# MecatronicaUSB/uwimageproc

Hardware: NVIDIA B200
Metric: chain_frames_per_s_4k (higher is better)
Workload: dtype u8 (histretch, aclahe) / int32+f64 (bgdehaze)

## Files before the change

### uwimageproc_b200/csrc/dehaze.cu

```cuda
#include <algorithm>

#include "common.cuh"

__global__ void fs_reset_kernel(FrameState* fs, int n) {
  int i = blockIdx.x * blockDim.x + threadIdx.x;
  if (i >= n) return;
  FrameState s;
  memset(&s, 0, sizeof(s));
  s.kmin = 255; s.kmax = 0;
  s.jmin_key[0] = s.jmin_key[1] = ~0ull;
  s.jmax_key[0] = s.jmax_key[1] = 0ull;
  s.rmin = 255; s.rmax = 0;
  s.yi_min = s.yj_min = 255; s.yi_max = s.yj_max = 0;
  s.omin_key = ~0ull; s.omax_key = 0ull;
  fs[i] = s;
}
int frame_state_reset(uwip_ctx* ctx, FrameState* fs, int n) {
  UWIP_LAUNCH(ctx, "fs_reset", fs_reset_kernel, cdiv(n, 128), 128, 0, fs, n);
  return UWIP_OK;
}
FrameState* frame_state_get(uwip_ctx* ctx, int n) { return (FrameState*)uwip_slot(ctx, SLOT_FSTATE, sizeof(FrameState) * (size_t)n); }

#include "gfmarch.cuh"

// ... 141 lines not shown
constexpr int WF_VR = WF_TY / 4, WF_CTAS = 3;
constexpr int WF_RB = 8;
constexpr int WF_PP = 84;
constexpr int WF_HP = 68;
constexpr int WF_HN = 16;

template <int N, bool MAX, int OFF, int M>
__device__ __forceinline__ void win15(const uint32_t (&p)[M], uint32_t (&o)[N]) {
  static_assert(OFF + N + 14 <= M, "window run");
  uint32_t a[N + 12], b[N + 6];
#pragma unroll
  for (int i = 0; i < N + 12; i++)
    a[i] = MAX ? __vimax3_u16x2(p[OFF + i], p[OFF + i + 1], p[OFF + i + 2]) : __vimin3_u16x2(p[OFF + i], p[OFF + i + 1], p[OFF + i + 2]);
#pragma unroll
  for (int i = 0; i < N + 6; i++) b[i] = MAX ? __vimax3_u16x2(a[i], a[i + 3], a[i + 6]) : __vimin3_u16x2(a[i], a[i + 3], a[i + 6]);
#pragma unroll
  for (int i = 0; i < N; i++) o[i] = MAX ? __vmaxu2(b[i], b[i + 6]) : __vminu2(b[i], b[i + 6]);
}

__device__ __forceinline__ void wf_cp_async8(void* smem, const void* gmem) {
  asm volatile("cp.async.ca.shared.global [%0], [%1], 8;" ::"r"((uint32_t)__cvta_generic_to_shared(smem)), "l"(gmem) : "memory");
}

template <bool FAST>
__device__ __forceinline__ uint32_t wf_emit_rows(const uint32_t (&mx0)[WF_VR], const uint32_t (&mx1)[WF_VR], const uint32_t (&mn0)[WF_VR],
                                                 const uint32_t* __restrict__ pc0, const uint32_t* __restrict__ pc1,
                                                 uint32_t* __restrict__ kqp, uint8_t* __restrict__ mgq, unsigned Wp, int nrows, int gy0, int H,
                                                 bool xt, bool inside, uint32_t km2) {
  uint32_t dmin2 = 0xffffffffu;
#pragma unroll
  for (int i = 0; i < WF_VR; i++) {
    if (!FAST && i >= nrows) break;
    const unsigned o = (unsigned)i * Wp;
    if (!FAST && !inside) { kqp[o] = 0u; mgq[o] = 0; continue; }
    const uint32_t t0 = pc0[i * WF_PP] - km2, t1 = pc1[i * WF_PP] - km2;
    uint32_t tn = mn0[i] - km2;
    if (!FAST) {
      const int gy = gy0 + i;
      if (xt || gy < WF_R || gy + WF_R >= H) tn = 0u;
    }
    kqp[o] = __byte_perm(__byte_perm(t0, t1, 0x4420), tn, 0x4210);
    mgq[o] = (uint8_t)(tn >> 16);
    dmin2 = __vminu2(dmin2, mx1[i] + 0x01000100u - mx0[i]);
  }
  return dmin2;
}

template <int CH>
__device__ __forceinline__ void wf_exact(const uint32_t (&mx0)[WF_VR], const uint32_t (&mx1)[WF_VR], int nrows, uint32_t target, int kmin,
                                         const double* s_nrm, unsigned idx0, unsigned W, double& bd, unsigned& bi) {
#pragma unroll
  for (int i = 0; i < WF_VR; i++) {
    if (i >= nrows) break;
    const uint32_t mr = mx1[i] & 0xffffu, mc = CH ? (mx0[i] >> 16) : (mx0[i] & 0xffffu);
    if (mr + 256u - mc == target) {
      const double d = s_nrm[mr - kmin] - s_nrm[mc - kmin];
      if (d < bd) { bd = d; bi = idx0 + (unsigned)i * W; }
    }
  }
}

__global__ void __launch_bounds__(256, WF_CTAS) window15_kernel(const uint8_t* __restrict__ src, int W, int H, int Wp,
                                                          const FrameState* __restrict__ fs, uint32_t* __restrict__ kq,
                                                          uint8_t* __restrict__ mgp, ArgPartial* __restrict__ partials) {
  extern __shared__ __align__(16) uint32_t s_w[];
  __shared__ double s_nrm[256];
  __shared__ uint32_t s_wmin[8];
  __shared__ int s_cnt[2];
  uint32_t* P0 = s_w;
  uint32_t* P1 = P0 + WF_RH * WF_PP;
  uint32_t* HX0 = P1 + WF_RH * WF_PP;
  uint32_t* HX1 = HX0 + WF_RH * WF_HP;
  uint32_t* HN0 = HX1 + WF_RH * WF_HP;
  const int f = blockIdx.z, tid = threadIdx.x, lane = tid & 31, warp = tid >> 5;
  const uint8_t* img = src + (size_t)f * W * H * 3;
  const int x0 = blockIdx.x * WF_TX, y0 = blockIdx.y * WF_TY;
  const int kmin = fs[f].kmin, range = (int)fs[f].kmax - kmin;
  s_nrm[tid] = (double)tid / (double)range;
  if (tid < 2) s_cnt[tid] = 0;
  uint32_t* RAW = HX0;
  const bool words = ((W & 3) == 0) && ((reinterpret_cast<uintptr_t>(img) & 3) == 0);
  const bool dwords = ((W & 7) == 0) && ((reinterpret_cast<uintptr_t>(img) & 7) == 0);
  if (dwords && x0 >= WF_RB && x0 - WF_RB + 80 <= W) {
    const uint2* col = reinterpret_cast<const uint2*>(img + (size_t)(x0 - WF_RB) * 3);
#pragma unroll
    for (int k = 0; k < (WF_RH + 7) / 8; k++) {
      const int ry = warp + 8 * k;
      if (ry < WF_RH && lane < 30) {
        const int y = min(max(y0 - WF_R + ry, 0), H - 1);
        wf_cp_async8(reinterpret_cast<uint2*>(RAW + ry * 64) + lane, col + (size_t)y * (W * 3 / 8) + lane);
      }
    }
    asm volatile("cp.async.wait_all;" ::: "memory");
    __syncthreads();
    for (int t = tid; t < WF_RH * 20; t += 256) {
      const int ry = t / 20, g = t - ry * 20;
      const uint32_t* w = RAW + ry * 64 + 3 * g;
      const uint32_t w0 = w[0], w1 = w[1], w2 = w[2];
      uint4 bg, rr;
      bg.x = __byte_perm(w0, 0u, 0x4140); bg.y = __byte_perm(w0, w1, 0x0403) & 0x00ff00ffu;
      bg.z = __byte_perm(w1, 0u, 0x4342); bg.w = __byte_perm(w2, 0u, 0x4241);
      rr.x = __byte_perm(w0, 0u, 0x4242); rr.y = __byte_perm(w1, 0u, 0x4141);
      rr.z = __byte_perm(w2, 0u, 0x4040); rr.w = __byte_perm(w2, 0u, 0x4343);
      *reinterpret_cast<uint4*>(P0 + ry * WF_PP + 4 * g) = bg;
      *reinterpret_cast<uint4*>(P1 + ry * WF_PP + 4 * g) = rr;
    }
  } else if (words) {
    const int xa = max(x0 - WF_RB, 0), xb = min(x0 - WF_RB + 79, W - 1);
    const int byte0 = (xa * 3) & ~3;
    const int nw = ((xb * 3 + 2) >> 2) - (byte0 >> 2) + 1;
#pragma unroll 4
    for (int idx = tid; idx < WF_RH * 64; idx += 256) {
      const int ry = idx >> 6, wi = idx & 63;
      if (wi < nw) {
        const int y = min(max(y0 - WF_R + ry, 0), H - 1);
        RAW[idx] = __ldg(reinterpret_cast<const uint32_t*>(img + (size_t)y * W * 3 + byte0) + wi);
      }
    }
    __syncthreads();
    if (tid < 240) {
      const int rx = tid % 80, rr = tid / 80;
      const int xc = min(max(x0 - WF_RB + rx, 0), W - 1);
      const uint8_t* rawb = reinterpret_cast<const uint8_t*>(RAW) + (xc * 3 - byte0);
#pragma unroll 7
      for (int ry = rr; ry < WF_RH; ry += 3) {
        const uint8_t* p = rawb + ry * 256;
        uint32_t b = p[0], g = p[1], r = p[2];
        P0[ry * WF_PP + rx] = b | (g << 16);
        P1[ry * WF_PP + rx] = r | (r << 16);
      }
    }
  } else if (tid < 240) {
    const int rx = tid % 80, rr = tid / 80;
    const int xc = min(max(x0 - WF_RB + rx, 0), W - 1);
    const uint8_t* col = img + (size_t)xc * 3;
#pragma unroll 7
    for (int ry = rr; ry < WF_RH; ry += 3) {
      const int y = min(max(y0 - WF_R + ry, 0), H - 1);
      const uint8_t* p = col + (size_t)y * W * 3;
      uint32_t b = __ldg(p), g = __ldg(p + 1), r = __ldg(p + 2);
      P0[ry * WF_PP + rx] = b | (g << 16);
      P1[ry * WF_PP + rx] = r | (r << 16);
    }
  }
  __syncthreads();
  if (tid < WF_RH * (WF_TX / WF_HN)) {
    const int ry = tid % WF_RH, j = tid / WF_RH;
    uint32_t p[WF_HN + 16], o[WF_HN];
    const uint4* r0 = reinterpret_cast<const uint4*>(P0 + ry * WF_PP + WF_HN * j);
#pragma unroll
    for (int q = 0; q < (WF_HN + 16) / 4; q++) { const uint4 v = r0[q]; p[4 * q] = v.x; p[4 * q + 1] = v.y; p[4 * q + 2] = v.z; p[4 * q + 3] = v.w; }
    win15<WF_HN, true, 1>(p, o);
    uint4* h0 = reinterpret_cast<uint4*>(HX0 + ry * WF_HP + WF_HN * j);
#pragma unroll
    for (int q = 0; q < WF_HN / 4; q++) h0[q] = make_uint4(o[4 * q], o[4 * q + 1], o[4 * q + 2], o[4 * q + 3]);
    win15<WF_HN, false, 1>(p, o);
    uint4* hn = reinterpret_cast<uint4*>(HN0 + ry * WF_HP + WF_HN * j);
#pragma unroll
    for (int q = 0; q < WF_HN / 4; q++) hn[q] = make_uint4(o[4 * q], o[4 * q + 1], o[4 * q + 2], o[4 * q + 3]);
    const uint4* r1 = reinterpret_cast<const uint4*>(P1 + ry * WF_PP + WF_HN * j);
#pragma unroll
    for (int q = 0; q < (WF_HN + 16) / 4; q++) { const uint4 v = r1[q]; p[4 * q] = v.x; p[4 * q + 1] = v.y; p[4 * q + 2] = v.z; p[4 * q + 3] = v.w; }
    win15<WF_HN, true, 1>(p, o);
    uint4* h1 = reinterpret_cast<uint4*>(HX1 + ry * WF_HP + WF_HN * j);
#pragma unroll
    for (int q = 0; q < WF_HN / 4; q++) h1[q] = make_uint4(o[4 * q], o[4 * q + 1], o[4 * q + 2], o[4 * q + 3]);
  }
  __syncthreads();
  const int x = tid & 63, run = tid >> 6;
  const int gx = x0 + x, ry0 = run * WF_VR, gy0 = y0 + ry0;
  const int nrows = gx < Wp ? min(WF_VR, H - gy0) : 0;
  const bool inside = gx < W;
  uint32_t mx0[WF_VR], mx1[WF_VR], dmin2 = 0xffffffffu;
  if (nrows > 0) {
    uint32_t p[WF_VR + 14], mn0[WF_VR];
#pragma unroll
    for (int i = 0; i < WF_VR + 14; i++) p[i] = HX0[(ry0 + i) * WF_HP + x];
    win15<WF_VR, true, 0>(p, mx0);
#pragma unroll
    for (int i = 0; i < WF_VR + 14; i++) p[i] = HX1[(ry0 + i) * WF_HP + x];
    win15<WF_VR, true, 0>(p, mx1);
#pragma unroll
    for (int i = 0; i < WF_VR + 14; i++) p[i] = HN0[(ry0 + i) * WF_HP + x];
    win15<WF_VR, false, 0>(p, mn0);
    const size_t pix0 = (size_t)f * Wp * H + (size_t)gy0 * Wp + gx;
    const uint32_t* pc0 = P0 + (ry0 + WF_R) * WF_PP + x + WF_RB;
    const uint32_t* pc1 = P1 + (ry0 + WF_R) * WF_PP + x + WF_RB;
    const uint32_t km2 = (uint32_t)kmin * 0x10001u;
    const bool xt = (gx < WF_R) || (gx + WF_R >= W);
    if (!xt && gy0 >= WF_R && gy0 + WF_VR - 1 + WF_R < H)
      dmin2 = wf_emit_rows<true>(mx0, mx1, mn0, pc0, pc1, kq + pix0, mgp + pix0, (unsigned)Wp, nrows, gy0, H, xt, inside, km2);
    else
      dmin2 = wf_emit_rows<false>(mx0, mx1, mn0, pc0, pc1, kq + pix0, mgp + pix0, (unsigned)Wp, nrows, gy0, H, xt, inside, km2);
  }
  {
    const uint32_t m0 = __reduce_min_sync(0xffffffffu, dmin2 & 0xffffu), m1 = __reduce_min_sync(0xffffffffu, dmin2 >> 16);
    if (lane == 0) s_wmin[warp] = m0 | (m1 << 16);
  }
  __syncthreads();
  double* cand_d = reinterpret_cast<double*>(HX0);
  unsigned* cand_i = reinterpret_cast<unsigned*>(cand_d + 512);
  uint32_t cm2 = s_wmin[0];
#pragma unroll
  for (int k = 1; k < 8; k++) cm2 = __vminu2(cm2, s_wmin[k]);
  if (inside && nrows > 0) {
    const unsigned idx0 = (unsigned)gy0 * (unsigned)W + (unsigned)gx;
    if ((dmin2 & 0xffffu) == (cm2 & 0xffffu)) {
      double bd = __longlong_as_double(0x7ff0000000000000ll); unsigned bi = 0xffffffffu;
      wf_exact<0>(mx0, mx1, nrows, cm2 & 0xffffu, kmin, s_nrm, idx0, (unsigned)W, bd, bi);
      const int slot = atomicAdd(&s_cnt[0], 1);
      cand_d[slot] = bd; cand_i[slot] = bi;
    }
    if ((dmin2 >> 16) == (cm2 >> 16)) {
      double bd = __longlong_as_double(0x7ff0000000000000ll); unsigned bi = 0xffffffffu;
      wf_exact<1>(mx0, mx1, nrows, cm2 >> 16, kmin, s_nrm, idx0, (unsigned)W, bd, bi);
      const int slot = atomicAdd(&s_cnt[1], 1);
      cand_d[256 + slot] = bd; cand_i[256 + slot] = bi;
    }
  }
  __syncthreads();
  if (warp < 2) {
    const int n = s_cnt[warp];
    double bd = __longlong_as_double(0x7ff0000000000000ll); unsigned bi = 0xffffffffu;
    for (int k = lane; k < n; k += 32) {
      const double d = cand_d[warp * 256 + k]; const unsigned i = cand_i[warp * 256 + k];
      if (lex_less(d, i, bd, bi)) { bd = d; bi = i; }
    }
#pragma unroll
    for (int d = 16; d > 0; d >>= 1) {
      const double od = __shfl_xor_sync(0xffffffffu, bd, d); const unsigned oi = __shfl_xor_sync(0xffffffffu, bi, d);
      if (lex_less(od, oi, bd, bi)) { bd = od; bi = oi; }
    }
    if (lane == 0) {
      ArgPartial* a = partials + ((size_t)f * gridDim.x * gridDim.y + blockIdx.y * gridDim.x + blockIdx.x);
      if (bi == 0xffffffffu) bd = __longlong_as_double(0x7ff0000000000000ll);
      if (warp == 0) { a->d0 = bd; a->i0 = bi; } else { a->d1 = bd; a->i1 = bi; }
    }
  }
}

__global__ void __launch_bounds__(256) bglight_finish_kernel(const uint8_t* __restrict__ src, int W, int H,
                                                             const ArgPartial* __restrict__ partials, int n_part, FrameState* fs,
                                                             int write_B, int write_Bt) {
  __shared__ ArgPartial s_part[8];
  int f = blockIdx.x;
  const ArgPartial* pp = partials + (size_t)f * n_part;
  double bd0 = __longlong_as_double(0x7ff0000000000000ll), bd1 = bd0;
  unsigned bi0 = 0xffffffffu, bi1 = 0xffffffffu;
  for (int i = threadIdx.x; i < n_part; i += 256) {
    ArgPartial a = pp[i];
    if (lex_less(a.d0, a.i0, bd0, bi0)) { bd0 = a.d0; bi0 = a.i0; }
    if (lex_less(a.d1, a.i1, bd1, bi1)) { bd1 = a.d1; bi1 = a.i1; }
  }
#pragma unroll
  for (int d = 16; d > 0; d >>= 1) {
    double o0 = __shfl_xor_sync(0xffffffffu, bd0, d), o1 = __shfl_xor_sync(0xffffffffu, bd1, d);
    unsigned j0 = __shfl_xor_sync(0xffffffffu, bi0, d), j1 = __shfl_xor_sync(0xffffffffu, bi1, d);
    if (lex_less(o0, j0, bd0, bi0)) { bd0 = o0; bi0 = j0; }
    if (lex_less(o1, j1, bd1, bi1)) { bd1 = o1; bi1 = j1; }
  }
  if ((threadIdx.x & 31) == 0) { ArgPartial a; a.d0 = bd0; a.d1 = bd1; a.i0 = bi0; a.i1 = bi1; s_part[threadIdx.x >> 5] = a; }
  __syncthreads();
  if (threadIdx.x == 0) {
    ArgPartial a = s_part[0];
    for (int k = 1; k < 8; k++) {
      ArgPartial b = s_part[k];
      if (lex_less(b.d0, b.i0, a.d0, a.i0)) { a.d0 = b.d0; a.i0 = b.i0; }
      if (lex_less(b.d1, b.i1, a.d1, a.i1)) { a.d1 = b.d1; a.i1 = b.i1; }
    }
    FrameState& s = fs[f];
    int kmin = s.kmin;
    double range = (double)((int)s.kmax - kmin);
    if (a.i0 == 0xffffffffu || a.i1 == 0xffffffffu) {
      a.i0 = a.i1 = 0;
      s.nan_flag = 1;
    }
    if (write_B) { s.idx0 = a.i0; s.idx1 = a.i1; }
    const uint8_t* img = src + (size_t)f * W * H * 3;
    for (int c = 0; c < 3; c++) {
      double v0 = (double)((int)img[(size_t)a.i0 * 3 + c] - kmin) / range;
      double v1 = (double)((int)img[(size_t)a.i1 * 3 + c] - kmin) / range;
      double b = (v0 + v1) / 2.0;
      if (write_B) s.B[c] = b;
      if (write_Bt) s.Bt[c] = b;
    }
  }
}

__global__ void traw_kernel(const uint32_t* __restrict__ kq, const uint8_t* __restrict__ mgp, int W, int H, int Wp,
                            const FrameState* __restrict__ fs, double* __restrict__ t_raw) {
  int x = blockIdx.x * blockDim.x + threadIdx.x, y = blockIdx.y;
  if (x >= W) return;
  const FrameState& s = fs[0];
  double range = (double)((int)s.kmax - (int)s.kmin);
  size_t pp = (size_t)y * Wp + x, pix = (size_t)y * W + x;
  int mb = (int)(kq[pp] >> 24), mg = (int)mgp[pp];
  t_raw[pix] = 1.0 - ((double)mb / range) / s.Bt[0];
  t_raw[(size_t)W * H + pix] = 1.0 - ((double)mg / range) / s.Bt[1];
}

#ifndef DZ_EW_CTAS
#define DZ_EW_CTAS 4
#endif
__global__ void __launch_bounds__(256, DZ_EW_CTAS) exposure_minmax_kernel(GfCommon g, int W, int H, int Wp, double* dbg_restored) {
  __shared__ ExpShared sh;
  int f = blockIdx.y;
  size_t n_pp = (size_t)Wp * H;
  exp_shared_init(&sh, g.fs[f], (double)W * (double)H);
  const uint32_t* kq = g.kq + (size_t)f * n_pp;
  const float* J = g.J + (size_t)f * 2 * n_pp;
  uint32_t* ycc = g.ycc + (size_t)f * n_pp;
  unsigned imn = 255, imx = 0, jmn = 255, jmx = 0;
  const int qpr = Wp / 4;
  const size_t n_q = (size_t)qpr * H;
  for (size_t qi = (size_t)blockIdx.x * 256 + threadIdx.x; qi < n_q; qi += (size_t)gridDim.x * 256) {
    int y = (int)(qi / qpr), x0 = (int)(qi - (size_t)y * qpr) * 4;
    size_t pp = (size_t)y * Wp + x0;
    uint4 kw = __ldg(reinterpret_cast<const uint4*>(kq + pp));
    float4 jb = __ldg(reinterpret_cast<const float4*>(J + pp)), jg = __ldg(reinterpret_cast<const float4*>(J + n_pp + pp));
    uint32_t out[4];
#pragma unroll
    for (int c = 0; c < 4; c++) {
      out[c] = 0;
      if (x0 + c >= W) continue;
      uint32_t w = quad_get(kw, c);
      uint32_t kb = w & 255u, kg = (w >> 8) & 255u, kr = (w >> 16) & 255u;
      int r8b = restored_byte(quad_get(jb, c), sh.fc, 0), r8g = restored_byte(quad_get(jg, c), sh.fc, 1), r8r = sh.rt.red8[kr];
      if (dbg_restored && f == 0) {
        size_t pix = (size_t)y * W + x0 + c;
        dbg_restored[pix * 3] = norm_j(quad_get(jb, c), sh.fc, 0); dbg_restored[pix * 3 + 1] = norm_j(quad_get(jg, c), sh.fc, 1);
        dbg_restored[pix * 3 + 2] = sh.rt.redN[kr];
      }
      int Yi, Cri, Cbi, Yj, Crj, Cbj;
      bgr2ycrcb_u8(sh.rt.i8[kb], sh.rt.i8[kg], sh.rt.i8[kr], Yi, Cri, Cbi);
      imn = min(imn, (unsigned)imin3(Yi, Cri, Cbi)); imx = max(imx, (unsigned)imax3(Yi, Cri, Cbi));
      bgr2ycrcb_u8(r8b, r8g, r8r, Yj, Crj, Cbj);
      jmn = min(jmn, (unsigned)imin3(Yj, Crj, Cbj)); jmx = max(jmx, (unsigned)imax3(Yj, Crj, Cbj));
      out[c] = (uint32_t)Yi | ((uint32_t)Cri << 8) | ((uint32_t)Cbi << 16) | ((uint32_t)Yj << 24);
    }
    *reinterpret_cast<uint4*>(ycc + pp) = make_uint4(out[0], out[1], out[2], out[3]);
  }
  imn = warp_reduce_min_u32(imn); imx = warp_reduce_max_u32(imx);
  jmn = warp_reduce_min_u32(jmn); jmx = warp_reduce_max_u32(jmx);
  if ((threadIdx.x & 31) == 0) {
    FrameState& s = g.fs[f];
    atomicMin(&s.yi_min, imn); atomicMax(&s.yi_max, imx);
    atomicMin(&s.yj_min, jmn); atomicMax(&s.yj_max, jmx);
  }
}

constexpr uint32_t GP_S_NAN = 0xffffffffu;
__global__ void __launch_bounds__(256) stab_kernel(const FrameState* __restrict__ fs, uint32_t* __restrict__ stab) {
  int f = blockIdx.y, gy = blockIdx.x, j = threadIdx.x;
  const FrameState& s = fs[f];
  double yi_rng = (double)((int)s.yi_max - (int)s.yi_min), yj_rng = (double)((int)s.yj_max - (int)s.yj_min);
  double yi = (double)gy / yi_rng, yj = (double)j / yj_rng;
  double yi2 = 0.3 * (yi * yi);
  const double S = (yj * yi + yi2) / (yj * yj + yi2);
  stab[(size_t)f * 65536 + gy * 256 + j] = (S == S) ? __double2uint_rn(fmin(S, GP_S_PMAX) * GP_PSCALE) : GP_S_NAN;
}

__global__ void __launch_bounds__(256) splane_kernel(GfCommon g, int H, int Wp) {
  int f = blockIdx.y;
  size_t n_pp = (size_t)Wp * H;
  const FrameState& s = g.fs[f];
  const uint32_t a = s.yi_min, b = s.yj_min;
  const uint32_t ysub = a | (a << 8) | (a << 16) | (b << 24);
  const uint32_t* ycc = g.ycc + (size_t)f * n_pp;
  const uint32_t* stab = g.stab + (size_t)f * 65536;
  uint32_t* sp = reinterpret_cast<uint32_t*>(g.splane) + (size_t)f * n_pp;
  const size_t n_q = n_pp / 4;
  bool nan_seen = false;
  for (size_t qi = (size_t)blockIdx.x * 256 + threadIdx.x; qi < n_q; qi += (size_t)gridDim.x * 256) {
    uint4 yw = __ldg(reinterpret_cast<const uint4*>(ycc) + qi);
    uint32_t o[4];
#pragma unroll
    for (int c = 0; c < 4; c++) {
      uint32_t w = quad_get(yw, c);
      const bool pad = (w & 255u) < a || (w >> 24) < b;
      w -= ysub;
      const uint32_t S = pad ? 0u : __ldg(stab + (((w & 255u) << 8) | (w >> 24)));
      if (S == GP_S_NAN) nan_seen = true;
      o[c] = (S == GP_S_NAN) ? 0u : S;
    }
    reinterpret_cast<uint4*>(sp)[qi] = make_uint4(o[0], o[1], o[2], o[3]);
  }
  if (__any_sync(0xffffffffu, nan_seen) && (threadIdx.x & 31) == 0) atomicOr(&g.fs[f].nan_flag, 1u);
}

__global__ void __launch_bounds__(256, DZ_EW_CTAS) final_kernel(GfCommon g, int W, int H, int Wp, uint8_t* __restrict__ dst, double* dbg_out, int32_t* __restrict__ flags) {
  __shared__ ExpShared sh;
  int f = blockIdx.y;
  size_t n_pp = (size_t)Wp * H;
  exp_shared_init(&sh, g.fs[f], (double)W * (double)H);
  const FrameState& s = g.fs[f];
  double omn = dunkey(s.omin_key), den = dunkey(s.omax_key) - omn;
  double scale = 255.0 / den;
  bool nan_frame = s.nan_flag != 0;
  if (flags && blockIdx.x == 0 && threadIdx.x == 0) flags[f] = nan_frame ? UWIP_FRAME_NAN : 0;
  const uint32_t* kq = g.kq + (size_t)f * n_pp;
  const float* J = g.J + (size_t)f * 2 * n_pp;
  const float* refS = g.refS + (size_t)f * n_pp;
  uint8_t* out = dst + (size_t)f * W * H * 3;
  const int qpr = Wp / 4;
  const size_t n_q = (size_t)qpr * H;
  const bool vec_ok = (W % 4 == 0) && ((reinterpret_cast<uintptr_t>(out) & 3) == 0);
  for (size_t qi = (size_t)blockIdx.x * 256 + threadIdx.x; qi < n_q; qi += (size_t)gridDim.x * 256) {
    int y = (int)(qi / qpr), x0 = (int)(qi - (size_t)y * qpr) * 4;
    size_t pp = (size_t)y * Wp + x0;
    uint4 kw = __ldg(reinterpret_cast<const uint4*>(kq + pp));
    float4 jb = __ldg(reinterpret_cast<const float4*>(J + pp)), jg = __ldg(reinterpret_cast<const float4*>(J + n_pp + pp));
    float4 qs = __ldg(reinterpret_cast<const float4*>(refS + pp));
    uint8_t b[12];
#pragma unroll
    for (int c = 0; c < 4; c++) {
      double rest[3];
      rest[0] = norm_j_fast(quad_get(jb, c), sh.fc, 0);
      rest[1] = norm_j_fast(quad_get(jg, c), sh.fc, 1);
      rest[2] = sh.rt.redN[(quad_get(kw, c) >> 16) & 255u];
      double q = (double)quad_get(qs, c);
#pragma unroll
      for (int ch = 0; ch < 3; ch++) {
        double v = (rest[ch] * q - omn) * scale;
        if (dbg_out && f == 0 && x0 + c < W) dbg_out[((size_t)y * W + x0 + c) * 3 + ch] = nan_frame ? __longlong_as_double(0x7ff8000000000000ll) : (rest[ch] * q - omn) / den;
        int bv = 0;
        if (!nan_frame && v == v && fabs(v) < 2.0e9) bv = min(max(__double2int_rn(v), 0), 255);
        b[c * 3 + ch] = (uint8_t)bv;
      }
    }
    uint8_t* o = out + ((size_t)y * W + x0) * 3;
    if (vec_ok) {
      uint32_t* o32 = reinterpret_cast<uint32_t*>(o);
      o32[0] = (uint32_t)b[0] | ((uint32_t)b[1] << 8) | ((uint32_t)b[2] << 16) | ((uint32_t)b[3] << 24);
      o32[1] = (uint32_t)b[4] | ((uint32_t)b[5] << 8) | ((uint32_t)b[6] << 16) | ((uint32_t)b[7] << 24);
      o32[2] = (uint32_t)b[8] | ((uint32_t)b[9] << 8) | ((uint32_t)b[10] << 16) | ((uint32_t)b[11] << 24);
    } else {
      for (int c = 0; c < 4 && x0 + c < W; c++) { o[c * 3] = b[c * 3]; o[c * 3 + 1] = b[c * 3 + 1]; o[c * 3 + 2] = b[c * 3 + 2]; }
    }
  }
}

int dehaze_strips(int w) {
  GfGeom g = gf_geometry(w, 4 * 40 + 2, 40);
  return cdiv(w, g.SW);
}
int dehaze_strips_narrow(int w) { return dehaze_gf1a_strips(w); }
int dehaze_sub_batch(const uwip_ctx* ctx, int n, int w, int cap) {
  cap = std::max(1, cap);
  if (n <= cap) return n;
  GfGeom g = gf_geometry(w, 4 * 40 + 2, 40);
  const long long sw = cdiv(w, g.SW), sn = dehaze_gf1a_strips(w), sms = std::max(1, ctx->sm_count);
  auto waves = [&](long long frames, long long strips) { return (double)((frames * strips + sms - 1) / sms) / (double)strips; };
  double best_cost = -1.0;
  int best = cap;
  for (int m = cap; m >= std::max(1, cap / 2); m--) {
    const int full = n / m, rem = n - full * m;
    double cost = full * (0.64 * waves(m, sw) + 0.36 * waves(m, sn)) + (rem ? 0.64 * waves(rem, sw) + 0.36 * waves(rem, sn) : 0.0);
    if (best_cost < 0.0 || cost < best_cost - 1e-9) { best_cost = cost; best = m; }
  }
  return best;
}

int dehaze_frames_dev(uwip_ctx* ctx, const uint8_t* d_src, uint8_t* d_dst, int n, int W, int H, const uwip_dehaze_params& p,
                      bool minmax_done, FrameState* fs, DehazeDebug* dbg, int32_t* d_flags) {
  UWIP_REQUIRE(ctx, n >= 1 && W >= 1 && H >= 1, "bad size");
  UWIP_REQUIRE(ctx, p.window >= 1 && p.window <= WK_MAXWIN, "window must be 1..33");
  UWIP_REQUIRE(ctx, p.radius >= 1 && p.radius <= 160, "radius must be 1..160");
  UWIP_REQUIRE(ctx, p.eps > 0.0 && p.tmin <= 1.0, "eps must be positive and tmin <= 1");
  UWIP_REQUIRE(ctx, (size_t)W * H < (1ull << 31), "frame too large");
  UWIP_REQUIRE(ctx, !dbg || n == 1, "stage outputs are single-frame");
  size_t n_px = (size_t)W * H;
  const int Wp = (W + 3) & ~3;
  size_t n_pp = (size_t)Wp * H;
  if (!minmax_done) {
    int want = (int)std::min<size_t>((n_px * 3 / 16 + 255) / 256, 1u << 16);
    int gxm = std::max(1, std::min(want, ctx->sm_count * 8 / n + 1));
    dim3 grid(gxm, n);
    UWIP_LAUNCH(ctx, "dz_minmax", minmax_kernel, grid, 256, 0, d_src, n_px * 3, fs);
  }
  uint32_t* d_kq = (uint32_t*)uwip_slot(ctx, SLOT_KQ, (size_t)n * n_pp * 4);
  uint8_t* d_mg = (uint8_t*)uwip_slot(ctx, SLOT_MPLANES, (size_t)n * n_pp);
  uint32_t* d_ycc = (uint32_t*)uwip_slot(ctx, SLOT_YCC, (size_t)n * n_pp * 4);
  uint32_t* d_stab = (uint32_t*)uwip_slot(ctx, SLOT_STAB, (size_t)n * 65536 * 4);
  float* d_sp = (float*)uwip_slot(ctx, SLOT_SPLANE, (size_t)n * n_pp * sizeof(float));
  dim3 gridw(cdiv(Wp, WK_TX), cdiv(H, WK_TY), n);
  dim3 gridf(cdiv(Wp, WF_TX), cdiv(H, WF_TY), n);
  int n_part = gridw.x * gridw.y, n_partf = gridf.x * gridf.y;
  ArgPartial* d_part = (ArgPartial*)uwip_slot(ctx, SLOT_PARTIALS, (size_t)n * std::max(n_part, n_partf) * sizeof(ArgPartial));
  float* d_ab = (float*)uwip_slot(ctx, SLOT_AB, (size_t)n * 8 * n_pp * sizeof(float));
  float* d_J = (float*)uwip_slot(ctx, SLOT_J, (size_t)n * 2 * n_pp * sizeof(float));
  float* d_refS = (float*)uwip_slot(ctx, SLOT_REFS, (size_t)n * n_pp * sizeof(float));
  if (!d_kq || !d_mg || !d_ycc || !d_stab || !d_sp || !d_part || !d_ab || !d_J || !d_refS) return UWIP_ERR_NOMEM;
  {
    const int wmax = p.window, wmin = WK_TWIN;
    if (wmax != WK_TWIN) {
      int PL = std::max(wmax / 2, wmin / 2), PR = std::max(wmax - 1 - wmax / 2, wmin - 1 - wmin / 2);
      int RW = WK_TX + PL + PR, RH = WK_TY + PL + PR;
      size_t smem = ((size_t)2 * RW * RH + (size_t)3 * RH * WK_TX) * 4;
      UWIP_CUDA(ctx, uwip_func_smem(ctx, FUNC_WINDOW, window_kernel, smem));
      UWIP_LAUNCH(ctx, "dz_window", window_kernel, gridw, WK_THREADS, smem, d_src, W, H, Wp, wmax, fs, d_kq, d_mg, d_part);
      UWIP_LAUNCH(ctx, "dz_bglight", bglight_finish_kernel, n, 256, 0, d_src, W, H, d_part, n_part, fs, 1, 0);
    }
    size_t smemf = ((size_t)2 * WF_RH * WF_PP + (size_t)3 * WF_RH * WF_HP) * 4;
    UWIP_CUDA(ctx, uwip_func_smem(ctx, FUNC_WINDOW15, window15_kernel, smemf));
    UWIP_LAUNCH(ctx, "dz_window", window15_kernel, gridf, 256, smemf, d_src, W, H, Wp, fs, d_kq, d_mg, d_part);
    UWIP_LAUNCH(ctx, "dz_bglight", bglight_finish_kernel, n, 256, 0, d_src, W, H, d_part, n_partf, fs, wmax == WK_TWIN ? 1 : 0, 1);
  }
  if (dbg && dbg->stop_after == 1) return UWIP_OK;
  if (dbg && dbg->t_raw) {
    dim3 g2(cdiv(W, 256), H);
    UWIP_LAUNCH(ctx, "dz_traw", traw_kernel, g2, 256, 0, d_kq, d_mg, W, H, Wp, fs, dbg->t_raw);
  }
  if (dbg && dbg->stop_after == 2) return UWIP_OK;

  GfCommon gc;
  gc.kq = d_kq; gc.mg = d_mg; gc.ycc = d_ycc; gc.stab = d_stab; gc.splane = d_sp; gc.ab = d_ab; gc.J = d_J; gc.refS = d_refS; gc.fs = fs;
  gc.eps = p.eps; gc.tmin = p.tmin; gc.dbg_tref = dbg ? dbg->t_ref : nullptr;
  UWIP_CHECK(dehaze_gf1a_launch(ctx, gc, n, W, H, p.radius));
  UWIP_CHECK(gp_launch<PipGF1b>(ctx, "dz_gf1b", FUNC_GF1B, gc, n, W, H, p.radius));
  if (dbg && dbg->stop_after == 3) return UWIP_OK;
  int gx = std::max(1, std::min((int)((n_pp / 4 + 1023) / 1024), std::max(1, ctx->sm_count * 24 / n)));
  dim3 grid_e(gx, n);
  UWIP_LAUNCH(ctx, "dz_exposure_minmax", exposure_minmax_kernel, grid_e, 256, 0, gc, W, H, Wp, dbg ? dbg->restored : (double*)nullptr);
  if (dbg && dbg->stop_after == 4) return UWIP_OK;
  dim3 grid_s(256, n);
  UWIP_LAUNCH(ctx, "dz_stab", stab_kernel, grid_s, 256, 0, fs, d_stab);
  UWIP_LAUNCH(ctx, "dz_splane", splane_kernel, grid_e, 256, 0, gc, H, Wp);
  UWIP_CHECK(gp_launch<PipGF2a>(ctx, "dz_gf2a", FUNC_GF2A, gc, n, W, H, p.radius));
  UWIP_CHECK(gp_launch<PipGF2b>(ctx, "dz_gf2b", FUNC_GF2B, gc, n, W, H, p.radius));
  UWIP_LAUNCH(ctx, "dz_final", final_kernel, grid_e, 256, 0, gc, W, H, Wp, d_dst, dbg ? dbg->out : (double*)nullptr, d_flags);
  return UWIP_OK;
}

__global__ void __launch_bounds__(256) box_rows_kernel(const double* __restrict__ src, double* __restrict__ dst, int W, int H, int r) {
  const int x = blockIdx.x * 256 + threadIdx.x, y = blockIdx.y;
  if (x >= W) return;
  const double* row = src + (size_t)y * W;
  double s = 0.0;
  for (int k = max(x - r, 0); k <= min(x + r, W - 1); k++) s += row[k];
  dst[(size_t)y * W + x] = s;
}
__global__ void __launch_bounds__(256) box_cols_kernel(const double* __restrict__ src, double* __restrict__ dst, int W, int H, int r) {
  const int x = blockIdx.x * 256 + threadIdx.x, y = blockIdx.y;
  if (x >= W) return;
  double s = 0.0;
  for (int k = max(y - r, 0); k <= min(y + r, H - 1); k++) s += src[(size_t)k * W + x];
  dst[(size_t)y * W + x] = s;
}
int boxfilter_f64_dev(uwip_ctx* ctx, const double* d_src, double* d_tmp, double* d_dst, int W, int H, int r) {
  UWIP_REQUIRE(ctx, W >= 1 && H >= 1 && r >= 0, "bad size");
  dim3 grid(cdiv(W, 256), H);
  UWIP_LAUNCH(ctx, "box_rows", box_rows_kernel, grid, 256, 0, d_src, d_tmp, W, H, r);
  UWIP_LAUNCH(ctx, "box_cols", box_cols_kernel, grid, 256, 0, (const double*)d_tmp, d_dst, W, H, r);
  return UWIP_OK;
}

__global__ void __launch_bounds__(256) gfq_pack_kernel(const uint8_t* __restrict__ guide, const double* __restrict__ p, int W, int H, int Wp,
                                                       uint32_t* __restrict__ ycc, uint32_t* __restrict__ sp, FrameState* fs) {
  const int x = blockIdx.x * 256 + threadIdx.x, y = blockIdx.y;
  if (x >= Wp) return;
  uint32_t g = 0, P = 0;
  bool bad = false;
  if (x < W) {
    const uint8_t* q = guide + ((size_t)y * W + x) * 3;
    g = (uint32_t)q[0] | ((uint32_t)q[1] << 8) | ((uint32_t)q[2] << 16);
    const double v = p[(size_t)y * W + x];
    bad = !(v >= 0.0 && v <= GP_S_PMAX);
    P = bad ? 0u : __double2uint_rn(v * GP_PSCALE);
  }
  ycc[(size_t)y * Wp + x] = g;
  sp[(size_t)y * Wp + x] = P;
  if (bad) atomicOr(&fs[0].nan_flag, 2u);
}
__global__ void gfq_state_kernel(FrameState* fs, int range) {
  FrameState& s = fs[0];
  s.yi_min = 0; s.yi_max = (unsigned)range; s.yj_min = 0; s.yj_max = (unsigned)range;
  s.kmin = 0; s.kmax = (unsigned)range;
}
int guided_filter_u8_dev(uwip_ctx* ctx, const uint8_t* d_guide, const double* d_p, double* d_q, int W, int H, int range, int r, double eps,
                         FrameState* fs) {
  UWIP_REQUIRE(ctx, W >= 1 && H >= 1 && r >= 1 && r <= 160 && range >= 1 && range <= 255 && eps > 0.0, "bad argument");
  const int Wp = (W + 3) & ~3;
  const size_t n_pp = (size_t)Wp * H;
  uint32_t* d_ycc = (uint32_t*)uwip_slot(ctx, SLOT_YCC, n_pp * 4);
  float* d_sp = (float*)uwip_slot(ctx, SLOT_SPLANE, n_pp * 4);
  float* d_ab = (float*)uwip_slot(ctx, SLOT_AB, 8 * n_pp * 4);
  if (!d_ycc || !d_sp || !d_ab) return UWIP_ERR_NOMEM;
  UWIP_CHECK(frame_state_reset(ctx, fs, 1));
  UWIP_LAUNCH(ctx, "gfq_state", gfq_state_kernel, 1, 1, 0, fs, range);
  dim3 grid(cdiv(Wp, 256), H);
  UWIP_LAUNCH(ctx, "gfq_pack", gfq_pack_kernel, grid, 256, 0, d_guide, d_p, W, H, Wp, d_ycc, reinterpret_cast<uint32_t*>(d_sp), fs);
  GfCommon gc;
  memset(&gc, 0, sizeof(gc));
  gc.ycc = d_ycc; gc.splane = d_sp; gc.ab = d_ab; gc.fs = fs; gc.eps = eps; gc.tmin = 0.0; gc.dbg_tref = d_q;
  UWIP_CHECK(gp_launch<PipGF2a>(ctx, "dz_gf2a", FUNC_GF2A, gc, 1, W, H, r));
  UWIP_CHECK(gp_launch<PipGFq>(ctx, "gfq_out", FUNC_GFQ, gc, 1, W, H, r));
  return UWIP_OK;
}

#if GP_TRACE
extern "C" int uwip_exp_trace(long long* out) {
  return (int)cudaMemcpyFromSymbol(out, gp_trace_buf, sizeof(gp_trace_buf));
}
#endif
```

### uwimageproc_b200/csrc/gfmarch.cuh

```cuda
#pragma once
#include <algorithm>

#include "common.cuh"

__device__ __forceinline__ double u2d(uint32_t u) { return __uint2double_rn(u); }
__device__ __forceinline__ double rcp_fast(double x) {
  double r;
  asm("rcp.approx.ftz.f64 %0, %1;" : "=d"(r) : "d"(x));
  double e = fma(-x, r, 1.0);
  r = fma(r, e, r);
  e = fma(-x, r, 1.0);
  r = fma(r, e, r);
  return r;
}

template <int G>
__device__ __forceinline__ double grid_round(double x) {
  const double M = 6755399441055744.0 / (double)(1ull << G);
  return (x + M) - M;
}

__device__ __forceinline__ void cp_async16(void* smem, const void* g) {
  unsigned a = (unsigned)__cvta_generic_to_shared(smem);
  asm volatile("cp.async.cg.shared.global [%0], [%1], 16;" ::"r"(a), "l"(g) : "memory");
}
__device__ __forceinline__ void cp_async8(void* smem, const void* g) {
  asm volatile("cp.async.ca.shared.global [%0], [%1], 8;" ::"r"((unsigned)__cvta_generic_to_shared(smem)), "l"(g) : "memory");
}
__device__ __forceinline__ void cp_async_wait_2() { asm volatile("cp.async.wait_group 2;" ::: "memory"); }
__device__ __forceinline__ void cp_async4(void* smem, const void* g) {
  unsigned a = (unsigned)__cvta_generic_to_shared(smem);
  asm volatile("cp.async.ca.shared.global [%0], [%1], 4;" ::"r"(a), "l"(g) : "memory");
}
__device__ __forceinline__ void cp_async_commit() { asm volatile("cp.async.commit_group;" ::: "memory"); }
__device__ __forceinline__ void cp_async_wait_all() { asm volatile("cp.async.wait_group 0;" ::: "memory"); }
__device__ __forceinline__ void mbar_init(uint64_t* bar, unsigned count) {
  unsigned a = (unsigned)__cvta_generic_to_shared(bar);
  asm volatile("mbarrier.init.shared::cta.b64 [%0], %1;" ::"r"(a), "r"(count) : "memory");
}
__device__ __forceinline__ void mbar_arrive_expect_tx(uint64_t* bar, unsigned bytes) {
  unsigned a = (unsigned)__cvta_generic_to_shared(bar);
  asm volatile("mbarrier.arrive.expect_tx.shared::cta.b64 _, [%0], %1;" ::"r"(a), "r"(bytes) : "memory");
}
__device__ __forceinline__ void mbar_wait(uint64_t* bar, unsigned parity) {
  unsigned a = (unsigned)__cvta_generic_to_shared(bar);
  asm volatile(
      "{\n\t.reg .pred p;\n\t"
      "WAIT_%=:\n\t"
      "mbarrier.try_wait.parity.shared::cta.b64 p, [%0], %1;\n\t"
      "@p bra DONE_%=;\n\t"
      "bra WAIT_%=;\n\t"
      "DONE_%=:\n\t}" ::"r"(a), "r"(parity) : "memory");
}
__device__ __forceinline__ void tma_bulk_g2s(void* smem, const void* g, unsigned bytes, uint64_t* bar) {
  unsigned d = (unsigned)__cvta_generic_to_shared(smem), b = (unsigned)__cvta_generic_to_shared(bar);
  asm volatile("cp.async.bulk.shared::cluster.global.mbarrier::complete_tx::bytes [%0], [%1], %2, [%3];" ::"r"(d), "l"(g), "r"(bytes), "r"(b) : "memory");
}

__device__ __forceinline__ void gf_build_M(const uint32_t* si, double N, double epsN2, double* M, double* Sd) {
  Sd[0] = u2d(si[0]); Sd[1] = u2d(si[1]); Sd[2] = u2d(si[2]);
  M[0] = fma(N, u2d(si[3]), -Sd[0] * Sd[0]) + epsN2;
  M[1] = fma(N, u2d(si[4]), -Sd[0] * Sd[1]);
  M[2] = fma(N, u2d(si[5]), -Sd[0] * Sd[2]);
  M[3] = fma(N, u2d(si[6]), -Sd[1] * Sd[1]) + epsN2;
  M[4] = fma(N, u2d(si[7]), -Sd[1] * Sd[2]);
  M[5] = fma(N, u2d(si[8]), -Sd[2] * Sd[2]) + epsN2;
}
__device__ __forceinline__ void gf_adjugate(const double* M, double* A, double& rdet) {
  A[0] = M[3] * M[5] - M[4] * M[4];
  A[1] = M[2] * M[4] - M[1] * M[5];
  A[2] = M[1] * M[4] - M[2] * M[3];
  A[3] = M[0] * M[5] - M[2] * M[2];
  A[4] = M[1] * M[2] - M[0] * M[4];
  A[5] = M[0] * M[3] - M[1] * M[1];
  double det = M[0] * A[0] + M[1] * A[1] + M[2] * A[2];
  rdet = rcp_fast(det);
}
__device__ __forceinline__ void gf_solve(const double* A, double rdet, const double* Sd, double N, double invN, double Sp,
                                         const double* Sip, double* a, double& b) {
  double C0 = fma(N, Sip[0], -Sd[0] * Sp), C1 = fma(N, Sip[1], -Sd[1] * Sp), C2 = fma(N, Sip[2], -Sd[2] * Sp);
  a[0] = (C0 * A[0] + C1 * A[1] + C2 * A[2]) * rdet;
  a[1] = (C0 * A[1] + C1 * A[3] + C2 * A[4]) * rdet;
  a[2] = (C0 * A[2] + C1 * A[4] + C2 * A[5]) * rdet;
  b = (Sp - a[0] * Sd[0] - a[1] * Sd[1] - a[2] * Sd[2]) * invN;
}

__device__ __forceinline__ float4 coef_pack(const double* a, double b) {
  return make_float4((float)grid_round<34>(a[0]), (float)grid_round<34>(a[1]), (float)grid_round<34>(a[2]), (float)grid_round<34>(b));
}

struct GfCommon {
  const uint32_t* kq;
  const uint8_t* mg;
  uint32_t* ycc;
  const uint32_t* stab;
  float* splane;
  float* ab;
  float* J;
  float* refS;
  FrameState* fs;
  double eps, tmin;
  double* dbg_tref;
};

struct GfGeom {
  int W, H, Wp;
  int r;
  int HL;
  int SW;
  int NQ;
  int seg_h;
  int fast;
};

struct FrameConst {
  int kmin, range;
  double B[3], Bt[3];
  double jmin[2], jinv[2], jrcp[2];
  int yi_min, yi_rng, yj_min, yj_rng;
};

__device__ __forceinline__ void load_frame_const(const FrameState& s, FrameConst& c) {
  c.kmin = s.kmin;
  c.range = (int)s.kmax - (int)s.kmin;
  c.B[0] = s.B[0]; c.B[1] = s.B[1]; c.B[2] = s.B[2];
  c.Bt[0] = s.Bt[0]; c.Bt[1] = s.Bt[1]; c.Bt[2] = s.Bt[2];
  for (int k = 0; k < 2; k++) {
    double mn = dunkey(s.jmin_key[k]), mx = dunkey(s.jmax_key[k]);
    c.jmin[k] = mn;
    c.jinv[k] = mx - mn;
    c.jrcp[k] = 1.0 / (mx - mn);
  }
  c.yi_min = s.yi_min; c.yi_rng = (int)s.yi_max - (int)s.yi_min;
  c.yj_min = s.yj_min; c.yj_rng = (int)s.yj_max - (int)s.yj_min;
}

struct RedTables {
  double redN[256];
  uint8_t red8[256];
  uint8_t i8[256];
};
__device__ __forceinline__ int trunc_u8(double v) {
  if (!(v == v)) return 0;
  int i = (int)v;
  return i & 0xff;
}
static __device__ void build_red_tables(const FrameState& s, const FrameConst& fc, double n_px, RedTables* rt, int tid, int nthreads) {
  double range = (double)fc.range;
  double mean_b = ((double)s.jsum_fix[0] * (1.0 / 4294967296.0) / n_px - fc.jmin[0]) / fc.jinv[0];
  double mean_g = ((double)s.jsum_fix[1] * (1.0 / 4294967296.0) / n_px - fc.jmin[1]) / fc.jinv[1];
  double avgRr = 1.5 - mean_b - mean_g;
  double mean_r = ((double)s.rsum / n_px) / range;
  double coef = avgRr / mean_r;
  double ra = ((double)s.rmin / range) * coef, rb = ((double)s.rmax / range) * coef;
  double rmn = fmin(ra, rb), rmx = fmax(ra, rb);
  for (int k = tid; k < 256; k += nthreads) {
    double nk = (double)k / range;
    double v = (nk * coef - rmn) / (rmx - rmn);
    rt->redN[k] = v;
    rt->red8[k] = (uint8_t)trunc_u8(v * 255.0);
    rt->i8[k] = (uint8_t)trunc_u8(nk * 255.0);
  }
}

struct ExpShared {
  RedTables rt;
  FrameConst fc;
};
static __device__ void exp_shared_init(ExpShared* sh, const FrameState& s, double n_px) {
  if (threadIdx.x == 0) load_frame_const(s, sh->fc);
  __syncthreads();
  build_red_tables(s, sh->fc, n_px, &sh->rt, threadIdx.x, blockDim.x);
  __syncthreads();
}
__device__ __forceinline__ double norm_j(float j, const FrameConst& fc, int c) { return ((double)j - fc.jmin[c]) / fc.jinv[c]; }
__device__ __forceinline__ double norm_j_fast(float j, const FrameConst& fc, int c) { return ((double)j - fc.jmin[c]) * fc.jrcp[c]; }
__device__ __forceinline__ int restored_byte(float j, const FrameConst& fc, int c) {
  double v = norm_j_fast(j, fc, c) * 255.0;
  if (fabs(v - rint(v)) < 1.0e-9 || !(v == v)) v = norm_j(j, fc, c) * 255.0;
  return trunc_u8(v);
}

__device__ __forceinline__ unsigned long long warp_min_u64(unsigned long long v) {
#pragma unroll
  for (int d = 16; d > 0; d >>= 1) { unsigned long long o = __shfl_xor_sync(0xffffffffu, v, d); v = o < v ? o : v; }
  return v;
}
__device__ __forceinline__ unsigned long long warp_max_u64(unsigned long long v) {
#pragma unroll
  for (int d = 16; d > 0; d >>= 1) { unsigned long long o = __shfl_xor_sync(0xffffffffu, v, d); v = o > v ? o : v; }
  return v;
}
__device__ __forceinline__ long long warp_sum_i64(long long v) {
#pragma unroll
  for (int d = 16; d > 0; d >>= 1) v += __shfl_xor_sync(0xffffffffu, v, d);
  return v;
}
__device__ __forceinline__ float warp_min_f32(float v) {
#pragma unroll
  for (int d = 16; d > 0; d >>= 1) v = fminf(v, __shfl_xor_sync(0xffffffffu, v, d));
  return v;
}
__device__ __forceinline__ float warp_max_f32(float v) {
#pragma unroll
  for (int d = 16; d > 0; d >>= 1) v = fmaxf(v, __shfl_xor_sync(0xffffffffu, v, d));
  return v;
}
__device__ __forceinline__ double warp_sum_f64(double v) {
#pragma unroll
  for (int d = 16; d > 0; d >>= 1) v += __shfl_xor_sync(0xffffffffu, v, d);
  return v;
}
__device__ __forceinline__ double warp_min_f64(double v) {
#pragma unroll
  for (int d = 16; d > 0; d >>= 1) v = fmin(v, __shfl_xor_sync(0xffffffffu, v, d));
  return v;
}
__device__ __forceinline__ double warp_max_f64(double v) {
#pragma unroll
  for (int d = 16; d > 0; d >>= 1) v = fmax(v, __shfl_xor_sync(0xffffffffu, v, d));
  return v;
}

__device__ __forceinline__ uint32_t quad_get(const uint4& v, int c) { return c == 0 ? v.x : (c == 1 ? v.y : (c == 2 ? v.z : v.w)); }
__device__ __forceinline__ float quad_get(const float4& v, int c) { return c == 0 ? v.x : (c == 1 ? v.y : (c == 2 ? v.z : v.w)); }


template <int NP>
__device__ __forceinline__ int coef_chunk(int gq, int c, int j) {
  if (NP == 8) return (2 * c + j) ^ (gq & 7);
  return c ^ ((gq >> 1) & 3);
}

#define GP_COEF_T int
#define GP_COEF_V4 int4
#define GP_COEF_PACK(a, b, cs) coef_pack_fix(a, b, (cs).sa, (cs).sb)
#include "gfpipe.cuh"

static GfGeom gf_geometry(int W, int H, int r) {
  GfGeom g;
  g.W = W; g.H = H; g.Wp = (W + 3) & ~3; g.r = r;
  g.HL = (r + 3) & ~3;
  int sw_max = std::min(4 * (GP_NTR - 1) - 2 * g.HL, GP_MAXSW);
  int strips = cdiv(W, sw_max);
  g.SW = (cdiv(W, strips) + 3) & ~3;
  g.NQ = 1 + (2 * g.HL + g.SW) / 4;
  g.seg_h = H;
  g.fast = (r % 4 == 0) ? 1 : 0;
  return g;
}

template <class P>
static int gp_launch(uwip_ctx* ctx, const char* tag, int func_id, const GfCommon& gc, int n, int W, int H, int r) {
  GfGeom gg = gf_geometry(W, H, r);
  int strips = cdiv(W, gg.SW);
  int slots = ctx->sm_count;
  int tasks = strips * n;
  int best = 1;
  double best_eff = 0.0;
  int max_segs = std::max(1, H / (4 * r + 2));
  for (int s = 1; s <= max_segs && s <= 64; s++) {
    int sh = cdiv(H, s), sc = cdiv(H, sh);
    double waves = (double)cdiv(tasks * sc, slots);
    double eff = ((double)tasks * sc / (waves * slots)) * ((double)sh / (double)(sh + 2 * r));
    if (eff > best_eff * 1.02) { best_eff = eff; best = s; }
  }
  gg.seg_h = cdiv(H, best);
  int segs = cdiv(H, gg.seg_h);
  static_assert(GpSmem<P>::bytes <= 227 * 1024, "shared memory");
  size_t smem = GpSmem<P>::bytes;
  UWIP_CUDA(ctx, uwip_func_smem(ctx, func_id, gp_kernel<P>, smem));
  dim3 grid(strips, segs, n);
  UWIP_LAUNCH(ctx, tag, gp_kernel<P>, grid, GP_THREADS, smem, gc, gg);
  return UWIP_OK;
}
```

Before: 1259.

## Replace per-pixel fp64 restored-byte math with exact float threshold-table lookup

Each block now precomputes, by binary search over float bit patterns, the exact float threshold at which each restored byte value begins for the blue and green channels. Per-pixel conversion then becomes a float scale-and-estimate plus two table compares instead of fp64 multiply, rint and fallback divide. The exposure loop also prefetches the next iteration's loads into registers, uses 32-bit indexing, and gets a template specialization that skips edge and debug handling when the width is unpadded. Min-blocks in launch bounds drops from 4 to 3. The cost is per-block setup work for the threshold search and more registers and shared memory per block.

```diff
diff --git a/uwimageproc_b200/csrc/dehaze.cu b/uwimageproc_b200/csrc/dehaze.cu
--- a/uwimageproc_b200/csrc/dehaze.cu
+++ b/uwimageproc_b200/csrc/dehaze.cu
@@ -467,31 +467,39 @@
 #ifndef DZ_EW_CTAS
 #define DZ_EW_CTAS 4
 #endif
-__global__ void __launch_bounds__(256, DZ_EW_CTAS) exposure_minmax_kernel(GfCommon g, int W, int H, int Wp, double* dbg_restored) {
-  __shared__ ExpShared sh;
-  int f = blockIdx.y;
-  size_t n_pp = (size_t)Wp * H;
-  exp_shared_init(&sh, g.fs[f], (double)W * (double)H);
-  const uint32_t* kq = g.kq + (size_t)f * n_pp;
-  const float* J = g.J + (size_t)f * 2 * n_pp;
-  uint32_t* ycc = g.ycc + (size_t)f * n_pp;
-  unsigned imn = 255, imx = 0, jmn = 255, jmx = 0;
-  const int qpr = Wp / 4;
-  const size_t n_q = (size_t)qpr * H;
-  for (size_t qi = (size_t)blockIdx.x * 256 + threadIdx.x; qi < n_q; qi += (size_t)gridDim.x * 256) {
-    int y = (int)(qi / qpr), x0 = (int)(qi - (size_t)y * qpr) * 4;
-    size_t pp = (size_t)y * Wp + x0;
-    uint4 kw = __ldg(reinterpret_cast<const uint4*>(kq + pp));
-    float4 jb = __ldg(reinterpret_cast<const float4*>(J + pp)), jg = __ldg(reinterpret_cast<const float4*>(J + n_pp + pp));
+template <bool EDGE>
+__device__ __forceinline__ void exposure_loop(const ExpShared& sh, const float (*T)[RB_TABLE], float jminf0, float scf0, float jminf1,
+                                              float scf1, const uint32_t* __restrict__ kq, const float* __restrict__ J,
+                                              uint32_t* __restrict__ ycc, size_t n_pp, int W, unsigned qpr, unsigned n_q,
+                                              double* dbg_restored, unsigned& imn, unsigned& imx, unsigned& jmn, unsigned& jmx) {
+  const unsigned stride = gridDim.x * 256;
+  unsigned qi = blockIdx.x * 256 + threadIdx.x;
+  uint4 kw = make_uint4(0, 0, 0, 0);
+  float4 jb = make_float4(0.f, 0.f, 0.f, 0.f), jg = jb;
+  if (qi < n_q) {
+    kw = __ldg(reinterpret_cast<const uint4*>(kq) + qi);
+    jb = __ldg(reinterpret_cast<const float4*>(J) + qi); jg = __ldg(reinterpret_cast<const float4*>(J + n_pp) + qi);
+  }
+  for (; qi < n_q; qi += stride) {
+    const unsigned qn = qi + stride;
+    uint4 kw_n = kw;
+    float4 jb_n = jb, jg_n = jg;
+    if (qn < n_q) {
+      kw_n = __ldg(reinterpret_cast<const uint4*>(kq) + qn);
+      jb_n = __ldg(reinterpret_cast<const float4*>(J) + qn); jg_n = __ldg(reinterpret_cast<const float4*>(J + n_pp) + qn);
+    }
+    int nvalid = 4;
+    if (EDGE) nvalid = min(4, W - (int)(qi % qpr) * 4);
     uint32_t out[4];
 #pragma unroll
     for (int c = 0; c < 4; c++) {
       out[c] = 0;
-      if (x0 + c >= W) continue;
+      if (EDGE && c >= nvalid) continue;
       uint32_t w = quad_get(kw, c);
       uint32_t kb = w & 255u, kg = (w >> 8) & 255u, kr = (w >> 16) & 255u;
-      int r8b = restored_byte(quad_get(jb, c), sh.fc, 0), r8g = restored_byte(quad_get(jg, c), sh.fc, 1), r8r = sh.rt.red8[kr];
-      if (dbg_restored && f == 0) {
+      int r8b = rb_lookup(quad_get(jb, c), jminf0, scf0, T[0]), r8g = rb_lookup(quad_get(jg, c), jminf1, scf1, T[1]), r8r = sh.rt.red8[kr];
+      if (EDGE && dbg_restored && blockIdx.y == 0) {
+        const int y = (int)(qi / qpr), x0 = (int)(qi % qpr) * 4;
         size_t pix = (size_t)y * W + x0 + c;
         dbg_restored[pix * 3] = norm_j(quad_get(jb, c), sh.fc, 0); dbg_restored[pix * 3 + 1] = norm_j(quad_get(jg, c), sh.fc, 1);
         dbg_restored[pix * 3 + 2] = sh.rt.redN[kr];
@@ -503,8 +511,31 @@
       jmn = min(jmn, (unsigned)imin3(Yj, Crj, Cbj)); jmx = max(jmx, (unsigned)imax3(Yj, Crj, Cbj));
       out[c] = (uint32_t)Yi | ((uint32_t)Cri << 8) | ((uint32_t)Cbi << 16) | ((uint32_t)Yj << 24);
     }
-    *reinterpret_cast<uint4*>(ycc + pp) = make_uint4(out[0], out[1], out[2], out[3]);
-  }
+    reinterpret_cast<uint4*>(ycc)[qi] = make_uint4(out[0], out[1], out[2], out[3]);
+    kw = kw_n; jb = jb_n; jg = jg_n;
+  }
+}
+
+__global__ void __launch_bounds__(256, 3) exposure_minmax_kernel(GfCommon g, int W, int H, int Wp, double* dbg_restored) {
+  __shared__ ExpShared sh;
+  __shared__ float s_T[2][RB_TABLE];
+  int f = blockIdx.y;
+  size_t n_pp = (size_t)Wp * H;
+  exp_shared_init(&sh, g.fs[f], (double)W * (double)H);
+  const double jmn0 = sh.fc.jmin[0], jmn1 = sh.fc.jmin[1], jmx0 = dunkey(g.fs[f].jmax_key[0]), jmx1 = dunkey(g.fs[f].jmax_key[1]);
+  if (threadIdx.x == 0) { s_T[0][0] = s_T[1][0] = -INFINITY; s_T[0][256] = s_T[1][256] = INFINITY; }
+  else { s_T[0][threadIdx.x] = rb_threshold(threadIdx.x, jmn0, jmx0); s_T[1][threadIdx.x] = rb_threshold(threadIdx.x, jmn1, jmx1); }
+  const float jminf0 = (float)jmn0, jminf1 = (float)jmn1, scf0 = rb_scale(jmn0, jmx0), scf1 = rb_scale(jmn1, jmx1);
+  __syncthreads();
+  const uint32_t* kq = g.kq + (size_t)f * n_pp;
+  const float* J = g.J + (size_t)f * 2 * n_pp;
+  uint32_t* ycc = g.ycc + (size_t)f * n_pp;
+  unsigned imn = 255, imx = 0, jmn = 255, jmx = 0;
+  const unsigned qpr = (unsigned)Wp / 4, n_q = qpr * (unsigned)H;
+  if (Wp != W || dbg_restored)
+    exposure_loop<true>(sh, s_T, jminf0, scf0, jminf1, scf1, kq, J, ycc, n_pp, W, qpr, n_q, dbg_restored, imn, imx, jmn, jmx);
+  else
+    exposure_loop<false>(sh, s_T, jminf0, scf0, jminf1, scf1, kq, J, ycc, n_pp, W, qpr, n_q, nullptr, imn, imx, jmn, jmx);
   imn = warp_reduce_min_u32(imn); imx = warp_reduce_max_u32(imx);
   jmn = warp_reduce_min_u32(jmn); jmx = warp_reduce_max_u32(jmx);
   if ((threadIdx.x & 31) == 0) {
diff --git a/uwimageproc_b200/csrc/gfmarch.cuh b/uwimageproc_b200/csrc/gfmarch.cuh
--- a/uwimageproc_b200/csrc/gfmarch.cuh
+++ b/uwimageproc_b200/csrc/gfmarch.cuh
@@ -2,6 +2,7 @@
 #include <algorithm>
 
 #include "common.cuh"
+#include "restored_byte.h"
 
 __device__ __forceinline__ double u2d(uint32_t u) { return __uint2double_rn(u); }
 __device__ __forceinline__ double rcp_fast(double x) {
@@ -140,11 +141,6 @@
   uint8_t red8[256];
   uint8_t i8[256];
 };
-__device__ __forceinline__ int trunc_u8(double v) {
-  if (!(v == v)) return 0;
-  int i = (int)v;
-  return i & 0xff;
-}
 static __device__ void build_red_tables(const FrameState& s, const FrameConst& fc, double n_px, RedTables* rt, int tid, int nthreads) {
   double range = (double)fc.range;
   double mean_b = ((double)s.jsum_fix[0] * (1.0 / 4294967296.0) / n_px - fc.jmin[0]) / fc.jinv[0];
@@ -173,13 +169,8 @@
   build_red_tables(s, sh->fc, n_px, &sh->rt, threadIdx.x, blockDim.x);
   __syncthreads();
 }
-__device__ __forceinline__ double norm_j(float j, const FrameConst& fc, int c) { return ((double)j - fc.jmin[c]) / fc.jinv[c]; }
-__device__ __forceinline__ double norm_j_fast(float j, const FrameConst& fc, int c) { return ((double)j - fc.jmin[c]) * fc.jrcp[c]; }
-__device__ __forceinline__ int restored_byte(float j, const FrameConst& fc, int c) {
-  double v = norm_j_fast(j, fc, c) * 255.0;
-  if (fabs(v - rint(v)) < 1.0e-9 || !(v == v)) v = norm_j(j, fc, c) * 255.0;
-  return trunc_u8(v);
-}
+__device__ __forceinline__ double norm_j(float j, const FrameConst& fc, int c) { return rb_norm(j, fc.jmin[c], fc.jinv[c]); }
+__device__ __forceinline__ double norm_j_fast(float j, const FrameConst& fc, int c) { return rb_norm_fast(j, fc.jmin[c], fc.jrcp[c]); }
 
 __device__ __forceinline__ unsigned long long warp_min_u64(unsigned long long v) {
 #pragma unroll
diff --git a/uwimageproc_b200/csrc/restored_byte.h b/uwimageproc_b200/csrc/restored_byte.h
--- /dev/null
+++ b/uwimageproc_b200/csrc/restored_byte.h
@@ -0,0 +1,65 @@
+#pragma once
+#include <math.h>
+#include <stdint.h>
+#include <string.h>
+
+#ifdef __CUDACC__
+#define RB_HD __host__ __device__
+#else
+#define RB_HD
+#endif
+
+constexpr int RB_TABLE = 257;
+
+RB_HD inline int trunc_u8(double v) {
+  if (!(v == v)) return 0;
+  int i = (int)v;
+  return i & 0xff;
+}
+RB_HD inline double rb_norm(float j, double jmin, double jinv) { return ((double)j - jmin) / jinv; }
+RB_HD inline double rb_norm_fast(float j, double jmin, double jrcp) { return ((double)j - jmin) * jrcp; }
+RB_HD inline int rb_byte(float j, double jmin, double jinv, double jrcp) {
+  double v = rb_norm_fast(j, jmin, jrcp) * 255.0;
+  if (fabs(v - rint(v)) < 1.0e-9 || !(v == v)) v = rb_norm(j, jmin, jinv) * 255.0;
+  return trunc_u8(v);
+}
+
+RB_HD inline uint32_t rb_fkey(float f) {
+  uint32_t u;
+  memcpy(&u, &f, 4);
+  return (u & 0x80000000u) ? ~u : (u | 0x80000000u);
+}
+RB_HD inline float rb_funkey(uint32_t k) {
+  const uint32_t u = (k & 0x80000000u) ? (k & 0x7fffffffu) : ~k;
+  float f;
+  memcpy(&f, &u, 4);
+  return f;
+}
+
+RB_HD inline float rb_threshold(int b, double jmin, double jmax) {
+  const double jinv = jmax - jmin, jrcp = 1.0 / (jmax - jmin);
+  const float lo_f = (float)jmin, hi_f = (float)jmax;
+  if (!(rb_byte(hi_f, jmin, jinv, jrcp) >= b)) return INFINITY;
+  uint32_t lo = rb_fkey(lo_f), hi = rb_fkey(hi_f);
+  if (rb_byte(lo_f, jmin, jinv, jrcp) >= b) return lo_f;
+  while (hi - lo > 1) {
+    const uint32_t mid = lo + (hi - lo) / 2;
+    if (rb_byte(rb_funkey(mid), jmin, jinv, jrcp) >= b) hi = mid; else lo = mid;
+  }
+  return rb_funkey(hi);
+}
+
+inline void rb_table(double jmin, double jmax, float* T) {
+  T[0] = -INFINITY;
+  for (int b = 1; b < 256; b++) T[b] = rb_threshold(b, jmin, jmax);
+  T[256] = INFINITY;
+}
+
+RB_HD inline int rb_lookup(float j, float jmin_f, float scale_f, const float* T) {
+  const float e = fminf(fmaxf((j - jmin_f) * scale_f, 0.0f), 255.0f);
+  int b = (int)e;
+  b += (j >= T[b + 1]) ? 1 : 0;
+  b -= (j < T[b]) ? 1 : 0;
+  return b;
+}
+RB_HD inline float rb_scale(double jmin, double jmax) { return (float)(255.0 / (jmax - jmin)); }
```

Result: faster. 1275 (median of 6 runs) (+1.3%).
